# mousecpn/Boosting-R-CNN

Hardware: AMD Instinct MI355X
Metric: images/sec (1333x800) Boosting R-CNN R50-PAFPN inference (higher is better)
Workload: dtype f32; 1 GPU; boosting_rcnn_r50_pafpn_1x_utdac.py inference (model(return_loss=False, rescale=True): device pass + result copy + bbox2result), batch 8 x 3x800x1344 per GPU, f32 MFMA conv stack, 1000 pre-NMS / 256 proposals per image, seeded synthetic weights; global_batch=8, parallelism=dp1

## Files before the change

boosting-r-cnn_amd/csrc/conv_common.h:

```cpp
#pragma once
#include "common.h"

namespace brcnn_conv {

typedef float f32x16 __attribute__((ext_vector_type(16)));
typedef float f32x4 __attribute__((ext_vector_type(4)));
typedef unsigned int u32x4 __attribute__((ext_vector_type(4)));

constexpr int OOB = 0x7fffffff;

constexpr int BK = 32, LDS_STRIDE = 36;

struct ConvParams {
    const float* x;
    const float* w;
    const float* scale;
    const float* shift;
    const float* residual;
    float* y;
    int batch, Cin, Cout, KH, KW, stride, pad;
    int M, K;
    int relu;
    int tiles_m, tiles_n;
    int pitch;
// ... 78 lines not shown
    return r;
}
template <int ET> __device__ __forceinline__ unsigned brcnn_pk2(brcnn_f32x2 v) { return ET ? brcnn_pk2h(v.x, v.y) : brcnn_pk2b(v.x, v.y); }
__device__ __forceinline__ unsigned brcnn_relu_pk(unsigned w, unsigned floor2) {
    const brcnn_i16x2 a = __builtin_bit_cast(brcnn_i16x2, w), f = __builtin_bit_cast(brcnn_i16x2, floor2);
    return __builtin_bit_cast(unsigned, __builtin_elementwise_max(a, f));
}

int conv1x1_stream_try(ConvParams& p, hipStream_t s, int f16);
int dispatch_conv_bf16(ConvParams& p, hipStream_t s);
int dispatch_conv_pp_bf16(ConvParams& p, hipStream_t s);
int dispatch_conv_pp128_bf16(ConvParams& p, hipStream_t s);
int sk_plan_pp(ConvParams& p, int slots, int bm, int bn, hipStream_t s);
int sk_plan_pp_f32(ConvParams& p, int slots, int bm, int bn, hipStream_t s);
int sk_plan_f32_tile(ConvParams& p, int per_cu, int cus, hipStream_t s);
float* conv_ws_wgrad_slabs(hipStream_t s);
float* wgrad_defer_slabs(hipStream_t s, size_t bytes, int* err);
void wgrad_defer_push(hipStream_t s, float* slab, float* dw, int tiles, int tiles_k, int slices, int group, int Cout, int K,
                      int kind);
unsigned* conv_ws_wgrad_counters(hipStream_t s);
int wgrad_pp_bf16_try(const void* x, const void* dy, void* dw, int batch, int num_segments, const int* heights_host,
                      const int* widths_host, int cin, int cout, int kh, int kw, int stride, int pad, hipStream_t stream,
                      int f16);
int dispatch_conv_pp_f32(ConvParams& p, hipStream_t s);

}
```

boosting-r-cnn_amd/csrc/conv_igemm_bf16.hip:

```cpp
#include <algorithm>
#include <mutex>
#include <vector>
#include "conv_common.h"
#include "policy.h"

namespace {
using namespace brcnn_conv;

typedef __bf16 bf16x8 __attribute__((ext_vector_type(8)));
typedef _Float16 f16x8 __attribute__((ext_vector_type(8)));
typedef __attribute__((address_space(3))) void* lds_ptr_t;
constexpr int BKE = 64;

__device__ __forceinline__ unsigned short f2bf(float v) { return brcnn_f2b(v); }
__device__ __forceinline__ float bf2f(unsigned short h) { return __uint_as_float(((unsigned)h) << 16); }
template <int ET> __device__ __forceinline__ float e2f(unsigned short h) { return ET ? brcnn_h2f(h) : bf2f(h); }
template <int ET> __device__ __forceinline__ unsigned short f2e(float v) { return ET ? brcnn_f2h(v) : f2bf(v); }
template <int ET> __device__ __forceinline__ unsigned pk2e(float lo, float hi) { return ET ? brcnn_pk2h(lo, hi) : brcnn_pk2b(lo, hi); }

template <int MT, int NT, bool RES, bool OUTF32, int WM, int WNW = 2, int ST = 2, int ET = 0, int MODE = 0, bool SK = false>
__global__ __launch_bounds__(64 * WM * WNW, (ST == 2 && MT * NT <= 4 && (WM * WNW == 4 || MT == 1)) ? 2 : 1) void conv_igemm_bf16_dma_kernel(ConvParams p) {
    constexpr int NW = WNW * WM;
    constexpr int BM = 32 * MT * WM, BN = 32 * NT * WNW;
    constexpr int AG = BM / 8 / NW;
// ... 1118 lines not shown
    const long long tiles = (long long)p.tiles_m * p.tiles_n;
    const int nk = p.K / 32;
    if (nk < 2 || (p.K % 32) || tiles < slots || tiles * nk >= 0x7fffffffLL) return 0;
    if ((size_t)slots * 64 * 64 * sizeof(float) > SK_WS_BYTES) return 0;
    std::lock_guard<std::mutex> lock(g_sk_mutex);
    SkStream* st = nullptr;
    int rc = sk_stream_state(s, &st);
    if (rc) return rc;
    const SkTable* tab = nullptr;
    rc = sk_table_ranges(tiles, nk, slots, &tab);
    if (rc) return rc == BRCNN_EINVAL ? 0 : rc;
    sk_fill(p, *st, *tab);
    return 0;
}

static int dispatch_conv_f16(ConvParams& p, hipStream_t s) {
    p.il = 0;
    if (brcnn::g_policy.bf16_tile == 0) {
        if (const int rc = conv1x1_stream_try(p, s, 1)) return rc < 0 ? rc : 0;
    }
    if (p.gstep) return launch2<1, 1, 4, 2, 2, 1>(p, s);
    if (brcnn::g_policy.bf16_tile == 8842 && pp128_ok(p)) return dispatch_conv_pp128_bf16(p, s);
    if (brcnn::g_policy.bf16_tile == 8844 && pp_ok(p)) return dispatch_conv_pp_bf16(p, s);
    if (pp128_wins(p)) return dispatch_conv_pp128_bf16(p, s);
    if (pp_wins(p)) return dispatch_conv_pp_bf16(p, s);
    const long long t22 = (long long)((p.M + 127) / 128) * ((p.Cout + 127) / 128);
    const long long t44 = (long long)((p.M + 255) / 256) * ((p.Cout + 255) / 256);
    const bool fill44 = p.Cout >= 256 && p.K >= 1024 && !p.residual && !p.out_f32 && !p.z_out && !p.tail_z && t44 >= 512 &&
                        (double)t44 / (double)(((t44 + 255) / 256) * 256) >= 0.85;
    if (fill44 && p.Cout > 128) return launch2<2, 2, 4, 4, 2, 1>(p, s);
// ... 62 lines not shown
```

boosting-r-cnn_amd/csrc/conv_winograd_f32.hip:

```cpp
#include "conv_common.h"
#include "policy.h"

namespace {
using namespace brcnn_conv;

typedef __attribute__((address_space(3))) void* lds_ptr_t;

struct WinoSegs {
    int nseg, batch;
    int H[BRCNN_MAX_LEVELS], W[BRCNN_MAX_LEVELS], TH[BRCNN_MAX_LEVELS], TW[BRCNN_MAX_LEVELS];
    int t0[BRCNN_MAX_LEVELS + 1];
    int r0[BRCNN_MAX_LEVELS + 1];
};

struct WinoTile { int seg, n, h, w; };
__device__ __forceinline__ WinoTile wino_tile(const WinoSegs& sg, int t) {
    int s = 0;
#pragma unroll
    for (int i = 1; i < BRCNN_MAX_LEVELS; i++)
        if (i < sg.nseg && t >= sg.t0[i]) s = i;
    const int l = t - sg.t0[s];
    const int per = sg.TH[s] * sg.TW[s];
    const int n = l / per, rem = l - n * per;
    const int th = rem / sg.TW[s];
// ... 90 lines not shown
#pragma unroll
        for (int b = 0; b < 4; b++)
            *reinterpret_cast<float4*>(vs + (size_t)(a * 4 + b) * xi_stride) = make_float4(d[a][b][0], d[a][b][1], d[a][b][2], d[a][b][3]);
}

struct WinoGemmParams {
    const float* v;
    const float* u;
    const float* scale;
    const float* shift;
    float* y;
    unsigned v_bytes, u_bytes;
    int tile0, nt, Cin, Cout, relu;
    int tiles_m, tiles_n;
    WinoSegs sg;
};

constexpr int WBM_MAX = 64;

__device__ __forceinline__ constexpr int wino_at(int a, int i) { return a == 0 ? (i < 3 ? 1 : 0) : (i == 0 ? 0 : (i == 1 ? 1 : -1)); }

template <int WBM, int WBN, int WNW>
__global__ __launch_bounds__(256, 2) void wino_gemm_kernel(WinoGemmParams p) {
#if defined(__HIP_DEVICE_COMPILE__)
    constexpr int NB = WBN / (32 * WNW);
    static_assert(WBM % 32 == 0 && (WBM / 32) * WNW == 4 && NB * 32 * WNW == WBN && (NB == 1 || NB == 2), "four waves of 32 x 32 NB");
    static_assert(2 * WBM * 32 + 2 * WBN * 32 >= 4 * 1024, "the read-out slabs live in the staging buffers");
    __shared__ __attribute__((aligned(16))) float smem[2 * WBM * 32 + 2 * WBN * 32];
    float* As = smem;
    float* Bs = smem + 2 * WBM * 32;
    const int tid = threadIdx.x;
    const int lane = tid & 63;
    const int wave = __builtin_amdgcn_readfirstlane(tid >> 6);
    const int wm = wave / WNW, wn = wave % WNW;
    const int li = lane & 31, lh = lane >> 5;

    const int tile = xcd_remap(blockIdx.x, p.tiles_m * p.tiles_n);
    const int tile_m = tile / p.tiles_n, tile_n = tile - tile_m * p.tiles_n;
    const int m0 = tile_m * WBM, n0 = tile_n * WBN;

    const __amdgpu_buffer_rsrc_t rsrc_v = __builtin_amdgcn_make_buffer_rsrc((void*)p.v, 0, (int)p.v_bytes, 0x00020000);
    const __amdgpu_buffer_rsrc_t rsrc_u = __builtin_amdgcn_make_buffer_rsrc((void*)p.u, 0, (int)p.u_bytes, 0x00020000);

    constexpr int AG = WBM / 8 / 4, BG = WBN / 8 / 4;
    const int rg = lane >> 3, pc = lane & 7;
    int a_off[AG], b_off[BG];
#pragma unroll
    for (int j = 0; j < AG; j++) {
        const int r = (wave * AG + j) * 8 + rg;
        const int t = m0 + r;
        a_off[j] = t < p.nt ? (t * p.Cin + (pc ^ ((r >> 1) & 7)) * 4) * 4 : -1;
    }
#pragma unroll
    for (int j = 0; j < BG; j++) {
        const int r = (wave * BG + j) * 8 + rg;
        const int co = n0 + r;
        b_off[j] = co < p.Cout ? (co * p.Cin + (pc ^ ((r >> 1) & 7)) * 4) * 4 : -1;
    }
    const int nk = p.Cin / 32;
    const int a_xi = p.nt * p.Cin * 4, b_xi = p.Cout * p.Cin * 4;
    int s_xi = 0, s_kc = 0;
    auto dma_step = [&](int buf) {
        const int ao = s_xi * a_xi + s_kc * 128, bo = s_xi * b_xi + s_kc * 128;
        if (++s_kc == nk) { s_kc = 0; s_xi++; }
#pragma unroll
        for (int j = 0; j < AG; j++) {
            float* dst = As + buf * WBM * 32 + (wave * AG + j) * 8 * 32;
            __builtin_amdgcn_raw_ptr_buffer_load_lds(rsrc_v, (lds_ptr_t)dst, 16, a_off[j] >= 0 ? a_off[j] + ao : OOB, 0, 0, 0);
        }
#pragma unroll
        for (int j = 0; j < BG; j++) {
            float* dst = Bs + buf * WBN * 32 + (wave * BG + j) * 8 * 32;
            __builtin_amdgcn_raw_ptr_buffer_load_lds(rsrc_u, (lds_ptr_t)dst, 16, b_off[j] >= 0 ? b_off[j] + bo : OOB, 0, 0, 0);
        }
    };

// ... 13 lines not shown
        if constexpr (NB == 2)
            asm volatile("s_waitcnt lgkmcnt(0)" : "+v"(av[slot]), "+v"(bv[slot][0]), "+v"(bv[slot][NB - 1]) :: "memory");
        else
            asm volatile("s_waitcnt lgkmcnt(0)" : "+v"(av[slot]), "+v"(bv[slot][0]) :: "memory");
    };

    f32x16 yacc[4][NB], tmp[NB];
#pragma unroll
    for (int q = 0; q < 4; q++)
#pragma unroll
        for (int b = 0; b < NB; b++)
#pragma unroll
            for (int r = 0; r < 16; r++) yacc[q][b][r] = 0.f;

    dma_step(0);
    asm volatile("s_waitcnt vmcnt(0)" ::: "memory");
    __syncthreads();
    int cur = 0;
    for (int xi = 0; xi < 16; xi++) {
#pragma unroll
        for (int b = 0; b < NB; b++)
#pragma unroll
            for (int r = 0; r < 16; r++) tmp[b][r] = 0.f;
        for (int kc = 0; kc < nk; kc++) {
            const unsigned a_cur = a_lane + cur * (WBM * 32 * 4);
            const unsigned b_cur = b_lane + cur * (WBN * 32 * 4);
            frag_read(0, a_cur + chb[0], b_cur + chb[0]);
            if (xi < 15 || kc + 1 < nk) dma_step(cur ^ 1);
            frag_wait(0);
#pragma unroll
            for (int kk = 0; kk < 4; kk++) {
                const int sl = kk & 1;
                if (kk + 1 < 4) frag_read(sl ^ 1, a_cur + chb[kk + 1], b_cur + chb[kk + 1]);
#pragma unroll
                for (int e = 0; e < 4; e++)
#pragma unroll
                    for (int b = 0; b < NB; b++)
                        tmp[b] = __builtin_amdgcn_mfma_f32_32x32x2f32(av[sl][e], bv[sl][b][e], tmp[b], 0, 0, 0);
                if (kk + 1 < 4) frag_wait(sl ^ 1);
            }
            asm volatile("s_waitcnt vmcnt(0)" ::: "memory");
            __syncthreads();
            cur ^= 1;
        }
        const int i = xi >> 2, j = xi & 3;
#pragma unroll
        for (int a = 0; a < 2; a++)
#pragma unroll
            for (int bq = 0; bq < 2; bq++) {
                const float c = (float)(wino_at(a, i) * wino_at(bq, j));
#pragma unroll
                for (int b = 0; b < NB; b++)
#pragma unroll
                    for (int r = 0; r < 16; r++) yacc[a * 2 + bq][b][r] = __builtin_fmaf(c, tmp[b][r], yacc[a * 2 + bq][b][r]);
            }
    }

    float* slab = smem + wave * 1024;
    const int vrow = lane >> 3, vcol = (lane & 7) * 4;
    long long prow[4];
    int pw[4], pflag[4];
#pragma unroll
    for (int it = 0; it < 4; it++) {
        const int tl = m0 + wm * 32 + it * 8 + vrow;
        prow[it] = -1; pw[it] = 0; pflag[it] = 0;
        if (tl < p.nt) {
            const WinoTile t = wino_tile(p.sg, p.tile0 + tl);
            const int H = p.sg.H[t.seg], W = p.sg.W[t.seg];
            prow[it] = ((long long)p.sg.r0[t.seg] + ((long long)t.n * H + t.h) * W + t.w) * p.Cout;
            pw[it] = W;
// ... 17 lines not shown
                slab[((r & 3) + 8 * (r >> 2) + 4 * lh) * 32 + li] = o + sh;
            }
            __builtin_amdgcn_s_waitcnt(0xc07f);
            __builtin_amdgcn_wave_barrier();
#pragma unroll
            for (int it = 0; it < 4; it++) {
                float4 o = *reinterpret_cast<const float4*>(slab + (it * 8 + vrow) * 32 + vcol);
                if (p.relu) { o.x = fmaxf(o.x, 0.f); o.y = fmaxf(o.y, 0.f); o.z = fmaxf(o.z, 0.f); o.w = fmaxf(o.w, 0.f); }
                const bool in_map = ((q & 1) == 0 || (pflag[it] & 1)) && ((q & 2) == 0 || (pflag[it] & 2));
                if (prow[it] >= 0 && in_map && cv < p.Cout)
                    *reinterpret_cast<float4*>(yout + prow[it] + (long long)((q >> 1) * pw[it] + (q & 1)) * p.Cout + cv) = o;
            }
            __builtin_amdgcn_s_waitcnt(0xc07f);
            __builtin_amdgcn_wave_barrier();
        }
    }
#endif
}

int wino_segs(WinoSegs& sg, int batch, int num_segments, const int* heights_host, const int* widths_host) {
    if (batch <= 0 || num_segments <= 0 || num_segments > BRCNN_MAX_LEVELS || !heights_host || !widths_host) return BRCNN_EINVAL;
    sg = {};
    sg.nseg = num_segments;
    sg.batch = batch;
    long long tiles = 0, rows = 0;
    for (int s = 0; s < num_segments; s++) {
        const int H = heights_host[s], W = widths_host[s];
        if (H <= 0 || W <= 0 || H >= 4096 || W >= 4096) return BRCNN_EINVAL;
        sg.H[s] = H; sg.W[s] = W; sg.TH[s] = (H + 1) / 2; sg.TW[s] = (W + 1) / 2;
        sg.t0[s] = (int)tiles; sg.r0[s] = (int)rows;
// ... 13 lines not shown
    if (cin <= 0 || wino_segs(sg, batch, num_segments, heights_host, widths_host)) return 0;
    return (size_t)16 * (size_t)sg.t0[num_segments] * (size_t)cin * sizeof(float);
}

BRCNN_API int brcnn_winograd_filter_f32(const void* w, void* u, int cout, int cin, int kh, int kw, int dtype, void* stream) {
    if (!w || !u || dtype != BRCNN_DT_F32 || kh != 3 || kw != 3 || cin <= 0 || cout <= 0 || (cin % 32) || (cout % 64) ||
        (long long)cout * cin * 64 >= 0x7fffffffLL)
        return BRCNN_EINVAL;
    hipLaunchKernelGGL(wino_filter_kernel, dim3((cout * cin + 255) / 256), dim3(256), 0, (hipStream_t)stream, (const float*)w,
                       (float*)u, cout, cin);
    BRCNN_LAUNCH_CHECK();
    return 0;
}

namespace {

int wino_run(const void* x, const void* u, const void* gn_stats, const float* gamma, const float* beta, int groups, int relu_in,
             const float* scale, const float* shift, int relu, void* y, void* workspace, size_t workspace_bytes, WinoGemmParams& p,
             int num_segments, int cin, int cout, int variant, void* stream) {
    const int tiles = p.sg.t0[num_segments];
    if ((long long)p.sg.r0[num_segments] * (cin > cout ? cin : cout) * 4 >= 0x7fffffffLL) return BRCNN_EINVAL;
    if (workspace_bytes < (size_t)16 * tiles * cin * sizeof(float)) return BRCNN_EINVAL;
    const int wbm = variant == 2 ? 32 : 64, wbn = variant == 3 ? 64 : 128;
    int chunks = brcnn::g_policy.f32_winograd_chunks;
    while ((long long)16 * ((tiles + chunks - 1) / chunks + WBM_MAX) * cin * 4 >= 0x7fffffffLL) chunks *= 2;
    const int per = ((tiles + chunks - 1) / chunks + WBM_MAX - 1) / WBM_MAX * WBM_MAX;
    hipStream_t s = (hipStream_t)stream;
    p.v = (const float*)workspace; p.u = (const float*)u; p.scale = scale; p.shift = shift; p.y = (float*)y;
    p.u_bytes = (unsigned)((long long)cout * cin * 64);
    p.Cin = cin; p.Cout = cout; p.relu = relu;
    p.tiles_n = (cout + wbn - 1) / wbn;
    for (int t0 = 0; t0 < tiles; t0 += per) {
        const int nt = tiles - t0 < per ? tiles - t0 : per;
        const long long th = (long long)nt * (cin >> 2);
        hipLaunchKernelGGL(wino_input_kernel, dim3((unsigned)((th + 255) / 256)), dim3(256), 0, s, (const float*)x, (float*)workspace,
                           p.sg, t0, nt, cin, (const double*)gn_stats, gamma, beta, groups, relu_in);
        BRCNN_LAUNCH_CHECK();
        p.tile0 = t0; p.nt = nt;
        p.v_bytes = (unsigned)((long long)16 * nt * cin * 4);
        p.tiles_m = (nt + wbm - 1) / wbm;
        const dim3 grid(p.tiles_m * p.tiles_n);
        if (variant == 2) hipLaunchKernelGGL((wino_gemm_kernel<32, 128, 4>), grid, dim3(256), 0, s, p);
        else if (variant == 3) hipLaunchKernelGGL((wino_gemm_kernel<64, 64, 2>), grid, dim3(256), 0, s, p);
        else hipLaunchKernelGGL((wino_gemm_kernel<64, 128, 2>), grid, dim3(256), 0, s, p);
        BRCNN_LAUNCH_CHECK();
    }
    return 0;
}

}

BRCNN_API int brcnn_conv3x3_winograd_f32_multi(const void* x, const void* u, const void* gn_stats, const float* gamma,
                                               const float* beta, int groups, int relu_in, const float* scale,
                                               const float* shift, int relu, void* y, void* workspace, size_t workspace_bytes,
                                               int batch, int num_segments, const int* heights_host, const int* widths_host,
                                               int cin, int cout, int kh, int kw, int stride, int pad, int dtype, void* stream) {
    if (!x || !u || !y || !workspace || dtype != BRCNN_DT_F32 || kh != 3 || kw != 3 || stride != 1 || pad != 1 || cin <= 0 ||
        cout <= 0 || (cin % 32) || (cout % 64) || (long long)cout * cin * 64 >= 0x7fffffffLL)
        return BRCNN_EINVAL;
    if (gn_stats && (!gamma || !beta || groups <= 0 || cin % groups)) return BRCNN_EINVAL;
    WinoGemmParams p = {};
    if (wino_segs(p.sg, batch, num_segments, heights_host, widths_host)) return BRCNN_EINVAL;
    const int st = wino_run(x, u, gn_stats, gamma, beta, groups, relu_in, scale, shift, relu, y, workspace, workspace_bytes, p,
                            num_segments, cin, cout, 1, stream);
    if (st) return st;
    brcnn::count(brcnn::g_counters.f32_winograd_launches);
    brcnn::g_counters.f32_winograd_tiles = p.sg.t0[num_segments];
    return 0;
}

BRCNN_API int brcnn_conv3x3_winograd_f32_layer(const void* x, const void* u, const float* scale, const float* shift, int relu,
                                               void* y, void* workspace, size_t workspace_bytes, int batch, int height, int width,
                                               int cin, int cout, int kh, int kw, int stride, int pad, int dtype, void* stream) {
    if (!x || !u || !y || !workspace || dtype != BRCNN_DT_F32 || kh != 3 || kw != 3 || stride != 1 || pad != 1 || cin <= 0 ||
        cout <= 0 || (cin % 32) || (cout % 64) || (long long)cout * cin * 64 >= 0x7fffffffLL)
        return BRCNN_EINVAL;
    WinoGemmParams p = {};
    if (wino_segs(p.sg, batch, 1, &height, &width)) return BRCNN_EINVAL;
    const int variant = brcnn::wino_gemm_variant(p.sg.t0[1], cout);
    const int st = wino_run(x, u, nullptr, nullptr, nullptr, 0, 0, scale, shift, relu, y, workspace, workspace_bytes, p, 1, cin,
                            cout, variant, stream);
    if (st) return st;
// ... 5 lines not shown
```

boosting-r-cnn_amd/csrc/policy.h:

```cpp
#pragma once

namespace brcnn {

struct Policy {
    int use_dma = 1;
    int force_wm = 0, force_nt = 0;
    int no_fast = 0;
    int pp_f32_n128 = 1;
    int pp_f32_mode = 1;
    int f32_tile_sk = 1;
    int f32_tile_sk_per_cu = 0;
    int f32_winograd = 1;
    int f32_winograd_chunks = 1;
    int f32_winograd_layer = 1;
    int f32_winograd_gemm = 0;

    int dcn_fused = 1;

    int bf16_tile = 0;
    int bf16_il = 0;
    int sk_mode = 1;
    int sk_par = 0;
    int pp_mode = 1;
    int pp128_mode = 1;
    int pp128_min_k = 4096;
    int pp128_max_t88 = 128;
    int sk_spin_limit = 1 << 24;
    int sk_drop_publish = 0;
    int stream_mode = 1;

// ... 28 lines not shown
    int stream1x1_launches = 0;
    int sk_chain_fills = 0;
    int sk_par_fills = 0;
    int sk_last_wgs = 0;
    int bf16_tile_launches = 0;
    int bf16_tile_rows = 0;
    int bf16_tile_cols = 0;
    int bf16_tile_waves = 0;
    int bf16_tile_stages = 0;
    int wgrad_bf16_tile_launches = 0;
    int wgrad_bf16_last_tile = 0;
    int f32_winograd_launches = 0;
    int f32_winograd_tiles = 0;
    int f32_winograd_layer_launches = 0;
    int f32_winograd_layer_variant = 0;
    int dcn_fused_launches = 0;
    int dcn_im2col_launches = 0;
    int roi_ordered_launches = 0;
    int roi_prepared_launches = 0;
    int roi_gather_chunked = 0;
    int roi_gather_last_ch = 0;
};
extern Counters g_counters;
inline void count(int& c) { c = (c + 1) & 0x7fffffff; }

int wino_layer_rule(int tiles, int cin, int cout);
int wino_gemm_rule(int tiles, int cout);
int wino_gemm_variant(int tiles, int cout);

}
```

boosting-r-cnn_amd/csrc/policy.hip:

```cpp
#include "common.h"
#include "policy.h"

__attribute__((require_constant_initialization)) brcnn::Policy brcnn::g_policy;
__attribute__((require_constant_initialization)) brcnn::Counters brcnn::g_counters;
using brcnn::g_counters, brcnn::g_policy;

BRCNN_API int brcnn_conv_set_tile(int wm, int nt) {
    if (wm == -1) { g_policy.use_dma = nt; return 0; }
    if (wm == -3) { if (nt < 0 || nt > 2) return BRCNN_EINVAL; g_policy.pp_f32_n128 = nt; return 0; }
    if (wm == -4) { if (nt != 0 && nt != 1) return BRCNN_EINVAL; g_policy.no_fast = nt; return 0; }
    if (wm == -5) { if (nt < 0 || nt > 2) return BRCNN_EINVAL; g_policy.f32_tile_sk = nt; return 0; }
    if (wm == -7) { if (nt < 0 || nt > 8) return BRCNN_EINVAL; g_policy.f32_tile_sk_per_cu = nt; return 0; }
    if (wm == -6) return nt == 0 ? g_counters.f32_tile_sk_launches : nt == 1 ? g_counters.f32_tile_sk_wgs : BRCNN_EINVAL;
    if (wm == -9) {
        int* const c[] = {&g_counters.pp_f32_launches, &g_counters.pp_f32_rows, &g_counters.pp_f32_cols, &g_counters.pp_bf16_launches,
                          &g_counters.pp128_bf16_launches, &g_counters.stream1x1_launches, &g_counters.sk_chain_fills,
                          &g_counters.sk_par_fills, &g_counters.sk_last_wgs, &g_counters.bf16_tile_launches, &g_counters.bf16_tile_rows,
                          &g_counters.bf16_tile_cols, &g_counters.bf16_tile_waves, &g_counters.bf16_tile_stages,
                          &g_counters.wgrad_bf16_tile_launches, &g_counters.wgrad_bf16_last_tile};
        const int count = (int)(sizeof(c) / sizeof(c[0]));
        if (nt < -1 || nt >= count) return BRCNN_EINVAL;
        if (nt == -1) {
            for (int* q : c) *q = 0;
            g_counters.f32_winograd_launches = g_counters.f32_winograd_tiles = 0;
            g_counters.dcn_fused_launches = g_counters.dcn_im2col_launches = 0;
            g_counters.f32_winograd_layer_launches = g_counters.f32_winograd_layer_variant = 0;
            return 0;
        }
        const int n = *c[nt];
        *c[nt] = 0;
        return n;
    }
    if (wm == -11) {
        if (nt == 0 || nt == 1) { g_policy.f32_winograd = nt; return 0; }
        if (nt == 2) return g_policy.f32_winograd;
        if (nt >= 11 && nt <= 18) { g_policy.f32_winograd_chunks = nt - 10; return 0; }
        return BRCNN_EINVAL;
    }
    if (wm == -12) {
        if (nt != 0 && nt != 1) return BRCNN_EINVAL;
        int& c = nt == 0 ? g_counters.f32_winograd_launches : g_counters.f32_winograd_tiles;
// ... 9 lines not shown
        const int n = c;
        c = 0;
        return n;
    }
    if (wm == -14) {
        if (nt >= 0 && nt <= 2) { g_policy.f32_winograd_layer = nt; return 0; }
        if (nt == 3) return g_policy.f32_winograd_layer;
        if (nt >= 20 && nt <= 23) { g_policy.f32_winograd_gemm = nt - 20; return 0; }
        if (nt == 24) return g_policy.f32_winograd_gemm;
        if (nt != 10 && nt != 11) return BRCNN_EINVAL;
        int& c = nt == 10 ? g_counters.f32_winograd_layer_launches : g_counters.f32_winograd_layer_variant;
        const int n = c;
        c = 0;
        return n;
    }
    if (wm == -2) { if (nt != 0 && nt != 1 && nt != 2 && nt != 128 && nt != 256) return BRCNN_EINVAL; g_policy.pp_f32_mode = nt; return 0; }
    if ((wm != 0 && wm != 1 && wm != 2 && wm != 4) || nt < 0 || nt > 2) return BRCNN_EINVAL;
    g_policy.force_wm = wm;
    g_policy.force_nt = nt;
    return 0;
}

int brcnn::wino_gemm_rule(int tiles, int cout) {
    (void)tiles; (void)cout;
    return 3;
}

int brcnn::wino_layer_rule(int tiles, int cin, int cout) {
    if (cin != cout) return 0;
    if (cin == 256) return tiles >= 5250;
    if (cin == 512) return tiles >= 444;
    return 0;
}

int brcnn::wino_gemm_variant(int tiles, int cout) {
    return g_policy.f32_winograd_gemm ? g_policy.f32_winograd_gemm : wino_gemm_rule(tiles, cout);
}

BRCNN_API int brcnn_winograd_layer_route(int tiles, int cin, int cout, int kh, int kw, int stride, int pad, int dilation,
                                         int groups, int dtype) {
    if (tiles <= 0 || cin <= 0 || cout <= 0 || kh != 3 || kw != 3 || stride != 1 || pad != 1 || dilation != 1 || groups != 1 ||
        (cin % 32) || (cout % 64) || dtype != BRCNN_DT_F32 || (long long)cout * cin * 64 >= 0x7fffffffLL)
        return 0;
    if (!g_policy.f32_winograd || !g_policy.f32_winograd_layer) return 0;
    if (g_policy.f32_winograd_layer == 2) return 1;
    return brcnn::wino_layer_rule(tiles, cin, cout);
}

BRCNN_API int brcnn_winograd_layer_gemm_variant(int tiles, int cout) { return brcnn::wino_gemm_variant(tiles, cout); }

BRCNN_API int brcnn_conv_set_tile_bf16(int mtnt) {
// ... 97 lines not shown
```

boosting-r-cnn_amd/lib.py:

```python
import ctypes
import os

_HERE = os.path.dirname(os.path.abspath(__file__))
LIB_PATH = os.environ.get('BRCNN_LIB_PATH') or os.path.join(_HERE, 'lib', 'libbrcnn_hip.so')
_lib = None

c_int, c_i64, c_f32, c_f64, c_ptr, c_size = (ctypes.c_int, ctypes.c_int64, ctypes.c_float,
                                             ctypes.c_double, ctypes.c_void_p, ctypes.c_size_t)

SIGNATURES = {
    'brcnn_version': (c_int, []),
    'brcnn_device_count': (c_int, []),
    'brcnn_roi_align_forward': (c_int, [c_ptr] * 5 + [c_int] * 7 + [c_f32] + [c_int] * 4 + [c_ptr]),
    'brcnn_roi_align_backward': (c_int, [c_ptr] * 3 + [c_int] * 7 + [c_f32] + [c_int] * 3 + [c_ptr]),
    'brcnn_roi_extract_forward': (c_int, [c_ptr] * 4 + [c_int] + [c_ptr] * 3 + [c_int] * 6 +
                                  [c_f32, c_int, c_ptr]),
    'brcnn_roi_extract_forward_ordered': (c_int, [c_ptr] * 4 + [c_int] + [c_ptr] * 3 + [c_int] * 6 +
                                          [c_f32, c_int, c_ptr, c_ptr]),
    'brcnn_roi_extract_prep_workspace_bytes': (c_size, [c_int]),
    'brcnn_roi_extract_order_min_rois': (c_int, []),
    'brcnn_roi_extract_forward_prepared': (c_int, [c_ptr] * 4 + [c_int] + [c_ptr] * 3 + [c_int] * 6 +
                                           [c_f32, c_int, c_ptr, c_ptr, c_size, c_ptr]),
    'brcnn_get_tuning': (c_int, [c_ptr]),
    'brcnn_set_tuning': (c_int, [c_ptr]),
# ... 16 lines not shown
    'brcnn_conv2d_nhwc': (c_int, [c_ptr] * 6 + [c_int] * 11 + [c_ptr]),
    'brcnn_conv_set_tile': (c_int, [c_int, c_int]),
    'brcnn_clock_probe': (c_int, [c_ptr, c_i64, c_ptr]),
    'brcnn_nms_prepare': (c_int, [c_ptr] * 9 + [c_int, c_int, c_ptr]),
    'brcnn_nms_collect': (c_int, [c_ptr] * 7 + [c_int, c_int, c_int, c_ptr]),
    'brcnn_conv2d_nhwc_scatter2': (c_int, [c_ptr] * 3 + [c_int] * 14 + [c_ptr]),
    'brcnn_conv2d_nhwc_multi': (c_int, [c_ptr] * 6 + [c_int, c_int, c_ptr, c_ptr] + [c_int] * 8 +
                                [c_ptr]),
    'brcnn_winograd_filter_f32': (c_int, [c_ptr, c_ptr] + [c_int] * 5 + [c_ptr]),
    'brcnn_conv3x3_winograd_f32_multi_workspace_bytes': (c_size, [c_int, c_int, c_ptr, c_ptr, c_int]),
    'brcnn_conv3x3_winograd_f32_multi': (c_int, [c_ptr] * 5 + [c_int, c_int, c_ptr, c_ptr, c_int, c_ptr, c_ptr, c_size,
                                                 c_int, c_int, c_ptr, c_ptr] + [c_int] * 7 + [c_ptr]),
    'brcnn_conv3x3_winograd_f32_layer': (c_int, [c_ptr] * 4 + [c_int, c_ptr, c_ptr, c_size] + [c_int] * 10 + [c_ptr]),
    'brcnn_winograd_layer_route': (c_int, [c_int] * 10),
    'brcnn_winograd_layer_gemm_variant': (c_int, [c_int, c_int]),
    'brcnn_groupnorm_nhwc_multi_stats': (c_int, [c_ptr, c_ptr, c_int, c_int, c_ptr, c_int, c_int, c_f32, c_int, c_ptr]),
    'brcnn_conv2d_dgrad_nhwc_multi': (c_int, [c_ptr] * 3 + [c_int, c_int] + [c_ptr] * 4 + [c_int] * 7 +
                                      [c_ptr]),
    'brcnn_conv2d_wgrad_nhwc_multi': (c_int, [c_ptr] * 3 + [c_int, c_int] + [c_ptr] * 2 + [c_int] * 7 +
                                      [c_ptr]),
    'brcnn_wgrad_defer_begin': (c_int, [c_ptr, c_ptr, c_size, c_int]),
    'brcnn_wgrad_defer_flush': (c_int, [c_ptr]),
    'brcnn_wgrad_defer_pending': (c_int, [c_ptr]),
    'brcnn_wgrad_defer_stats': (c_int, [c_ptr, c_ptr, c_ptr]),
    'brcnn_stem_workspace_bytes': (c_size, [c_int, c_int, c_int]),
    'brcnn_stem7x7s2_nchw': (c_int, [c_ptr] * 6 + [c_int] * 6 + [c_ptr]),
    'brcnn_stem7x7s2_pool_nchw': (c_int, [c_ptr] * 5 + [c_int] * 5 + [c_ptr]),
    'brcnn_bottleneck_tail_f32': (c_int, [c_ptr] * 9 + [c_int] * 3 + [c_ptr]),
    'brcnn_bottleneck_tail_16': (c_int, [c_ptr] * 9 + [c_int] * 4 + [c_ptr]),
    'brcnn_conv_set_tile_bf16': (c_int, [c_int]),
# ... 202 lines not shown
```

include/brcnn_hip.h:

```cpp
#ifndef BRCNN_HIP_H
#define BRCNN_HIP_H

#include <stddef.h>
#include <stdint.h>

#ifdef __cplusplus
extern "C" {
#endif

#define BRCNN_LAYOUT_NCHW 0
#define BRCNN_LAYOUT_NHWC 1

#define BRCNN_DT_F32 0
#define BRCNN_DT_BF16 1
#define BRCNN_DT_BF16_OUT_F32 2
#define BRCNN_DT_F16 3
#define BRCNN_DT_F16_OUT_F32 4

#define BRCNN_MAX_LEVELS 8
#define BRCNN_MAX_IMAGES 64

int brcnn_version(void);

int brcnn_clock_probe(int64_t *out2, int64_t wall_ticks_100mhz, void *stream);
// ... 141 lines not shown
int brcnn_winograd_filter_f32(const void *w, void *u, int cout, int cin, int kh, int kw, int dtype, void *stream);
size_t brcnn_conv3x3_winograd_f32_multi_workspace_bytes(int batch, int num_segments, const int *heights_host,
                                                        const int *widths_host, int cin);
int brcnn_conv3x3_winograd_f32_multi(const void *x, const void *u, const void *gn_stats, const float *gamma,
                                     const float *beta, int groups, int relu_in, const float *scale,
                                     const float *shift, int relu, void *y, void *workspace, size_t workspace_bytes,
                                     int batch, int num_segments, const int *heights_host, const int *widths_host,
                                     int cin, int cout, int kh, int kw, int stride, int pad, int dtype, void *stream);

int brcnn_conv3x3_winograd_f32_layer(const void *x, const void *u, const float *scale, const float *shift, int relu,
                                     void *y, void *workspace, size_t workspace_bytes, int batch, int height, int width,
                                     int cin, int cout, int kh, int kw, int stride, int pad, int dtype, void *stream);
int brcnn_winograd_layer_route(int tiles, int cin, int cout, int kh, int kw, int stride, int pad, int dilation,
                               int groups, int dtype);
int brcnn_winograd_layer_gemm_variant(int tiles, int cout);

int brcnn_conv2d_nhwc_grouped(const void *x, const void *w_tiles, const float *scale,
                              const float *shift, const void *residual, void *y, int batch,
                              int height, int width, int cin, int cout, int kh, int kw, int stride,
                              int pad, int window, int relu, int dtype, void *stream);
int brcnn_conv2d_dgrad_nhwc_grouped(const void *dy, const void *w_t_tiles, void *dx, int batch,
                                    int in_height, int in_width, int out_height, int out_width, int cin,
                                    int cout, int kh, int kw, int stride, int pad, int window, int dtype,
                                    void *stream);
int brcnn_conv2d_wgrad_nhwc_grouped(const void *x, const void *dy, void *dw_tiles, int batch, int height,
                                    int width, int cin, int cout, int kh, int kw, int stride, int pad,
                                    int window, int dtype, void *stream);

int brcnn_conv2d_dgrad_nhwc_multi(const void *dy, const void *w_t, void *dx, int batch,
                                  int num_segments, const int *in_heights_host,
// ... 321 lines not shown
```

Measured before the change: 394.3 images/sec.

## Add stream-K persistent scheduling and optional three-stage ring to Winograd f32 GEMM

```diff
diff --git a/boosting-r-cnn_amd/csrc/conv_common.h b/boosting-r-cnn_amd/csrc/conv_common.h
--- a/boosting-r-cnn_amd/csrc/conv_common.h
+++ b/boosting-r-cnn_amd/csrc/conv_common.h
@@ -116,6 +116,8 @@
 int sk_plan_pp(ConvParams& p, int slots, int bm, int bn, hipStream_t s);
 int sk_plan_pp_f32(ConvParams& p, int slots, int bm, int bn, hipStream_t s);
 int sk_plan_f32_tile(ConvParams& p, int per_cu, int cus, hipStream_t s);
+struct SkRangePlan { int wgs; const int4* items; float* ws; unsigned* flags; unsigned epoch; unsigned* err; int spin_limit; };
+int sk_plan_ranges(SkRangePlan& k, long long tiles, int nk, int slots, size_t slot_bytes, hipStream_t s);
 float* conv_ws_wgrad_slabs(hipStream_t s);
 float* wgrad_defer_slabs(hipStream_t s, size_t bytes, int* err);
 void wgrad_defer_push(hipStream_t s, float* slab, float* dw, int tiles, int tiles_k, int slices, int group, int Cout, int K,
diff --git a/boosting-r-cnn_amd/csrc/conv_igemm_bf16.hip b/boosting-r-cnn_amd/csrc/conv_igemm_bf16.hip
--- a/boosting-r-cnn_amd/csrc/conv_igemm_bf16.hip
+++ b/boosting-r-cnn_amd/csrc/conv_igemm_bf16.hip
@@ -1156,6 +1156,27 @@
     return 0;
 }
 
+int sk_plan_ranges(SkRangePlan& k, long long tiles, int nk, int slots, size_t slot_bytes, hipStream_t s) {
+    k = {};
+    if (int e = sk_take_error()) return e;
+    if (brcnn::g_policy.sk_mode == 0 || slots <= 0 || slots > SK_MAX_SLOTS) return 0;
+    if (sk_capturing(s)) return 0;
+    if (nk < 2 || tiles < slots || tiles * nk >= 0x7fffffffLL) return 0;
+    if ((size_t)slots * slot_bytes > SK_WS_BYTES) return 0;
+    std::lock_guard<std::mutex> lock(g_sk_mutex);
+    SkStream* st = nullptr;
+    int rc = sk_stream_state(s, &st);
+    if (rc) return rc;
+    const SkTable* tab = nullptr;
+    rc = sk_table_ranges(tiles, nk, slots, &tab);
+    if (rc) return rc == BRCNN_EINVAL ? 0 : rc;
+    ConvParams p = {};
+    sk_fill(p, *st, *tab);
+    k.wgs = p.sk_wgs; k.items = p.sk_items; k.ws = p.sk_ws; k.flags = p.sk_flags; k.epoch = p.sk_epoch; k.err = p.sk_err;
+    k.spin_limit = p.sk_spin_limit;
+    return 0;
+}
+
 static int dispatch_conv_f16(ConvParams& p, hipStream_t s) {
     p.il = 0;
     if (brcnn::g_policy.bf16_tile == 0) {
diff --git a/boosting-r-cnn_amd/csrc/conv_winograd_f32.hip b/boosting-r-cnn_amd/csrc/conv_winograd_f32.hip
--- a/boosting-r-cnn_amd/csrc/conv_winograd_f32.hip
+++ b/boosting-r-cnn_amd/csrc/conv_winograd_f32.hip
@@ -128,28 +128,32 @@
     int tile0, nt, Cin, Cout, relu;
     int tiles_m, tiles_n;
     WinoSegs sg;
+    const int4* sk_items;
+    float* sk_ws;
+    unsigned* sk_flags;
+    unsigned sk_epoch;
+    unsigned* sk_err;
+    int sk_spin_limit;
 };
 
 constexpr int WBM_MAX = 64;
 
 __device__ __forceinline__ constexpr int wino_at(int a, int i) { return a == 0 ? (i < 3 ? 1 : 0) : (i == 0 ? 0 : (i == 1 ? 1 : -1)); }
 
-template <int WBM, int WBN, int WNW>
-__global__ __launch_bounds__(256, 2) void wino_gemm_kernel(WinoGemmParams p) {
+template <int WBM, int WBN, int WNW, bool PERS, int RING>
+__device__ __forceinline__ void wino_gemm_item(const WinoGemmParams& p, float* smem, const int tile, const int xb_, const int xe_,
+                                               const int slot) {
 #if defined(__HIP_DEVICE_COMPILE__)
     constexpr int NB = WBN / (32 * WNW);
-    static_assert(WBM % 32 == 0 && (WBM / 32) * WNW == 4 && NB * 32 * WNW == WBN && (NB == 1 || NB == 2), "four waves of 32 x 32 NB");
-    static_assert(2 * WBM * 32 + 2 * WBN * 32 >= 4 * 1024, "the read-out slabs live in the staging buffers");
-    __shared__ __attribute__((aligned(16))) float smem[2 * WBM * 32 + 2 * WBN * 32];
+    const int xb = PERS ? xb_ : 0, xe = PERS ? xe_ : 16;
     float* As = smem;
-    float* Bs = smem + 2 * WBM * 32;
+    float* Bs = smem + RING * WBM * 32;
     const int tid = threadIdx.x;
     const int lane = tid & 63;
     const int wave = __builtin_amdgcn_readfirstlane(tid >> 6);
     const int wm = wave / WNW, wn = wave % WNW;
     const int li = lane & 31, lh = lane >> 5;
 
-    const int tile = xcd_remap(blockIdx.x, p.tiles_m * p.tiles_n);
     const int tile_m = tile / p.tiles_n, tile_n = tile - tile_m * p.tiles_n;
     const int m0 = tile_m * WBM, n0 = tile_n * WBN;
 
@@ -173,7 +177,7 @@
     }
     const int nk = p.Cin / 32;
     const int a_xi = p.nt * p.Cin * 4, b_xi = p.Cout * p.Cin * 4;
-    int s_xi = 0, s_kc = 0;
+    int s_xi = xb, s_kc = 0;
     auto dma_step = [&](int buf) {
         const int ao = s_xi * a_xi + s_kc * 128, bo = s_xi * b_xi + s_kc * 128;
         if (++s_kc == nk) { s_kc = 0; s_xi++; }
@@ -217,19 +221,76 @@
             for (int r = 0; r < 16; r++) yacc[q][b][r] = 0.f;
 
     dma_step(0);
+    if constexpr (RING == 3) {
+        if ((xe - xb) * nk > 1) dma_step(1);
+    }
+    if constexpr (PERS) {
+        if (xb > 0) {
+            if (tid == 0) {
+                int spins = 0;
+                while (__hip_atomic_load(p.sk_flags + slot, __ATOMIC_RELAXED, __HIP_MEMORY_SCOPE_AGENT) != p.sk_epoch &&
+                       ++spins < p.sk_spin_limit)
+                    __builtin_amdgcn_s_sleep(4);
+                if (spins >= p.sk_spin_limit)
+                    __hip_atomic_store(p.sk_err, p.sk_epoch | 0x80000000u, __ATOMIC_RELAXED, __HIP_MEMORY_SCOPE_SYSTEM);
+                __builtin_amdgcn_fence(__ATOMIC_ACQUIRE, "agent");
+            }
+            __syncthreads();
+            const f32x4* src = reinterpret_cast<const f32x4*>(p.sk_ws) + (size_t)slot * (WBM * WBN) + wave * 64 + lane;
+#pragma unroll
+            for (int q = 0; q < 4; q++)
+#pragma unroll
+                for (int b = 0; b < NB; b++)
+#pragma unroll
+                    for (int g = 0; g < 4; g++) {
+                        const f32x4 v = src[((q * NB + b) * 4 + g) * 256];
+                        yacc[q][b][4 * g + 0] = v.x; yacc[q][b][4 * g + 1] = v.y;
+                        yacc[q][b][4 * g + 2] = v.z; yacc[q][b][4 * g + 3] = v.w;
+                    }
+#pragma unroll
+            for (int q = 0; q < 4; q++)
+#pragma unroll
+                for (int b = 0; b < NB; b++) asm volatile("" : "+v"(yacc[q][b]));
+        }
+    }
     asm volatile("s_waitcnt vmcnt(0)" ::: "memory");
     __syncthreads();
     int cur = 0;
-    for (int xi = 0; xi < 16; xi++) {
+    [[maybe_unused]] int left = (xe - xb) * nk;
+    for (int xi = xb; xi < xe; xi++) {
 #pragma unroll
         for (int b = 0; b < NB; b++)
 #pragma unroll
             for (int r = 0; r < 16; r++) tmp[b][r] = 0.f;
+        if constexpr (RING == 3) {
+            for (int kc = 0; kc < nk; kc++, left--) {
+                if (left > 1) asm volatile("s_waitcnt vmcnt(%0)" ::"n"(AG + BG) : "memory");
+                else asm volatile("s_waitcnt vmcnt(0)" ::: "memory");
+                __syncthreads();
+                const unsigned a_cur = a_lane + cur * (WBM * 32 * 4);
+                const unsigned b_cur = b_lane + cur * (WBN * 32 * 4);
+                frag_read(0, a_cur + chb[0], b_cur + chb[0]);
+                if (left > 2) dma_step(cur == 0 ? 2 : cur - 1);
+                frag_wait(0);
+#pragma unroll
+                for (int kk = 0; kk < 4; kk++) {
+                    const int sl = kk & 1;
+                    if (kk + 1 < 4) frag_read(sl ^ 1, a_cur + chb[kk + 1], b_cur + chb[kk + 1]);
+#pragma unroll
+                    for (int e = 0; e < 4; e++)
+#pragma unroll
+                        for (int b = 0; b < NB; b++)
+                            tmp[b] = __builtin_amdgcn_mfma_f32_32x32x2f32(av[sl][e], bv[sl][b][e], tmp[b], 0, 0, 0);
+                    if (kk + 1 < 4) frag_wait(sl ^ 1);
+                }
+                cur = cur == 2 ? 0 : cur + 1;
+            }
+        } else
         for (int kc = 0; kc < nk; kc++) {
             const unsigned a_cur = a_lane + cur * (WBM * 32 * 4);
             const unsigned b_cur = b_lane + cur * (WBN * 32 * 4);
             frag_read(0, a_cur + chb[0], b_cur + chb[0]);
-            if (xi < 15 || kc + 1 < nk) dma_step(cur ^ 1);
+            if (xi < xe - 1 || kc + 1 < nk) dma_step(cur ^ 1);
             frag_wait(0);
 #pragma unroll
             for (int kk = 0; kk < 4; kk++) {
@@ -257,6 +318,32 @@
 #pragma unroll
                     for (int r = 0; r < 16; r++) yacc[a * 2 + bq][b][r] = __builtin_fmaf(c, tmp[b][r], yacc[a * 2 + bq][b][r]);
             }
+    }
+
+    if constexpr (RING == 3) __syncthreads();
+    if constexpr (PERS) {
+        if (xe < 16) {
+            f32x4* dst = reinterpret_cast<f32x4*>(p.sk_ws) + (size_t)slot * (WBM * WBN) + wave * 64 + lane;
+#pragma unroll
+            for (int q = 0; q < 4; q++)
+#pragma unroll
+                for (int b = 0; b < NB; b++)
+#pragma unroll
+                    for (int g = 0; g < 4; g++) {
+                        f32x4 v;
+                        v.x = yacc[q][b][4 * g + 0]; v.y = yacc[q][b][4 * g + 1];
+                        v.z = yacc[q][b][4 * g + 2]; v.w = yacc[q][b][4 * g + 3];
+                        dst[((q * NB + b) * 4 + g) * 256] = v;
+                    }
+            asm volatile("s_waitcnt vmcnt(0)" ::: "memory");
+            __syncthreads();
+            if (tid == 0) {
+                __builtin_amdgcn_fence(__ATOMIC_RELEASE, "agent");
+                asm volatile("s_waitcnt vmcnt(0)" ::: "memory");
+                __hip_atomic_store(p.sk_flags + slot, p.sk_epoch, __ATOMIC_RELAXED, __HIP_MEMORY_SCOPE_AGENT);
+            }
+            return;
+        }
     }
 
     float* slab = smem + wave * 1024;
@@ -304,6 +391,29 @@
             __builtin_amdgcn_s_waitcnt(0xc07f);
             __builtin_amdgcn_wave_barrier();
         }
+    }
+#endif
+}
+
+template <int WBM, int WBN, int WNW, bool PERS = false, int RING = 2>
+__global__ __launch_bounds__(256, 2) void wino_gemm_kernel(WinoGemmParams p) {
+#if defined(__HIP_DEVICE_COMPILE__)
+    static_assert(WBM % 32 == 0 && (WBM / 32) * WNW == 4 && (WBN == 32 * WNW || WBN == 64 * WNW), "four waves of 32 x 32 NB");
+    static_assert(RING == 2 || RING == 3, "two or three LDS stages");
+    static_assert(RING * (WBM * 32 + WBN * 32) >= 4 * 1024, "the read-out slabs live in the staging buffers");
+    __shared__ __attribute__((aligned(16))) float smem[RING * (WBM * 32 + WBN * 32)];
+    if constexpr (PERS) {
+        const int4 range = p.sk_items[blockIdx.x];
+        const int first = __builtin_amdgcn_readfirstlane(range.x), count = __builtin_amdgcn_readfirstlane(range.y);
+        for (int i = 0; i < count; i++) {
+            if (i > 0) __syncthreads();
+            const int4 item = p.sk_items[first + i];
+            wino_gemm_item<WBM, WBN, WNW, true, RING>(p, smem, __builtin_amdgcn_readfirstlane(item.x),
+                                                __builtin_amdgcn_readfirstlane(item.y), __builtin_amdgcn_readfirstlane(item.z),
+                                                __builtin_amdgcn_readfirstlane(item.w));
+        }
+    } else {
+        wino_gemm_item<WBM, WBN, WNW, false, RING>(p, smem, xcd_remap(blockIdx.x, p.tiles_m * p.tiles_n), 0, 16, 0);
     }
 #endif
 }
@@ -347,6 +457,64 @@
 }
 
 namespace {
+
+int g_wino_cus = 0;
+template <int WBM, int WBN, int WNW, int RING>
+int wino_occupancy(int& occ) {
+    static int cached = -1;
+    if (cached < 0) {
+        int n = 0;
+        BRCNN_HIP_CHECK(hipOccupancyMaxActiveBlocksPerMultiprocessor(&n, (const void*)wino_gemm_kernel<WBM, WBN, WNW, true, RING>, 256, 0));
+        if (g_wino_cus == 0) {
+            int dev = 0;
+            hipDeviceProp_t prop;
+            BRCNN_HIP_CHECK(hipGetDevice(&dev));
+            BRCNN_HIP_CHECK(hipGetDeviceProperties(&prop, dev));
+            g_wino_cus = prop.multiProcessorCount;
+        }
+        cached = n;
+    }
+    occ = cached;
+    return 0;
+}
+
+template <int RING>
+int wino_occupancy_of(int variant, int& occ) {
+    return variant == 2 ? wino_occupancy<32, 128, 4, RING>(occ) : variant == 3 ? wino_occupancy<64, 64, 2, RING>(occ)
+                                                                               : wino_occupancy<64, 128, 2, RING>(occ);
+}
+
+int wino_plan(WinoGemmParams& p, int variant, int ring, hipStream_t s, int& wgs) {
+    wgs = 0;
+    const int mode = brcnn::g_policy.f32_winograd_sk;
+    if (mode == 0) return 0;
+    int occ = 0;
+    if (const int rc = ring == 3 ? wino_occupancy_of<3>(variant, occ) : wino_occupancy_of<2>(variant, occ)) return rc;
+    const int cus = g_wino_cus;
+    const long long tiles = (long long)p.tiles_m * p.tiles_n;
+    int per_cu = occ;
+    if (brcnn::g_policy.f32_winograd_sk_per_cu > 0 && brcnn::g_policy.f32_winograd_sk_per_cu < per_cu) per_cu = brcnn::g_policy.f32_winograd_sk_per_cu;
+    if (per_cu <= 0 || cus <= 0) return 0;
+    if (tiles < (long long)per_cu * cus) per_cu = tiles / cus > 1 ? (int)(tiles / cus) : 1;
+    if (mode == 1 && !brcnn::wino_persistent_rule(tiles > 0x7fffffffLL ? 0x7fffffff : (int)tiles, 16, cus, per_cu)) return 0;
+    long long slots = (long long)per_cu * cus;
+    if (brcnn::g_policy.f32_winograd_sk_wgs > 0 && brcnn::g_policy.f32_winograd_sk_wgs < slots) slots = brcnn::g_policy.f32_winograd_sk_wgs;
+    const int wbm = variant == 2 ? 32 : 64, wbn = variant == 3 ? 64 : 128;
+    SkRangePlan k;
+    if (const int rc = sk_plan_ranges(k, tiles, 16, (int)slots, (size_t)4 * wbm * wbn * sizeof(float), s)) return rc;
+    if (k.wgs <= 0) return 0;
+    p.sk_items = k.items; p.sk_ws = k.ws; p.sk_flags = k.flags; p.sk_epoch = k.epoch; p.sk_err = k.err;
+    p.sk_spin_limit = k.spin_limit;
+    wgs = k.wgs;
+    return 0;
+}
+
+template <bool PERS, int RING>
+void wino_launch(int variant, const dim3& grid, hipStream_t s, const WinoGemmParams& p) {
+    if (variant == 2) hipLaunchKernelGGL((wino_gemm_kernel<32, 128, 4, PERS, RING>), grid, dim3(256), 0, s, p);
+    else if (variant == 3) hipLaunchKernelGGL((wino_gemm_kernel<64, 64, 2, PERS, RING>), grid, dim3(256), 0, s, p);
+    else hipLaunchKernelGGL((wino_gemm_kernel<64, 128, 2, PERS, RING>), grid, dim3(256), 0, s, p);
+}
 
 int wino_run(const void* x, const void* u, const void* gn_stats, const float* gamma, const float* beta, int groups, int relu_in,
              const float* scale, const float* shift, int relu, void* y, void* workspace, size_t workspace_bytes, WinoGemmParams& p,
@@ -372,10 +540,22 @@
         p.tile0 = t0; p.nt = nt;
         p.v_bytes = (unsigned)((long long)16 * nt * cin * 4);
         p.tiles_m = (nt + wbm - 1) / wbm;
+        const int ring = brcnn::g_policy.f32_winograd_ring ? brcnn::g_policy.f32_winograd_ring
+                                                           : brcnn::wino_ring_rule(p.tiles_m * p.tiles_n, cin);
+        brcnn::g_counters.f32_winograd_last_ring = ring;
+        int wgs = 0;
+        if (const int rc = wino_plan(p, variant, ring, s, wgs)) return rc;
+        if (wgs > 0) {
+            if (ring == 3) wino_launch<true, 3>(variant, dim3(wgs), s, p);
+            else wino_launch<true, 2>(variant, dim3(wgs), s, p);
+            BRCNN_LAUNCH_CHECK();
+            brcnn::count(brcnn::g_counters.f32_winograd_sk_launches);
+            brcnn::g_counters.f32_winograd_sk_last_wgs = wgs;
+            continue;
+        }
         const dim3 grid(p.tiles_m * p.tiles_n);
-        if (variant == 2) hipLaunchKernelGGL((wino_gemm_kernel<32, 128, 4>), grid, dim3(256), 0, s, p);
-        else if (variant == 3) hipLaunchKernelGGL((wino_gemm_kernel<64, 64, 2>), grid, dim3(256), 0, s, p);
-        else hipLaunchKernelGGL((wino_gemm_kernel<64, 128, 2>), grid, dim3(256), 0, s, p);
+        if (ring == 3) wino_launch<false, 3>(variant, grid, s, p);
+        else wino_launch<false, 2>(variant, grid, s, p);
         BRCNN_LAUNCH_CHECK();
     }
     return 0;
@@ -394,11 +574,14 @@
     if (gn_stats && (!gamma || !beta || groups <= 0 || cin % groups)) return BRCNN_EINVAL;
     WinoGemmParams p = {};
     if (wino_segs(p.sg, batch, num_segments, heights_host, widths_host)) return BRCNN_EINVAL;
+    const int variant = brcnn::g_policy.f32_winograd_tower_gemm ? brcnn::g_policy.f32_winograd_tower_gemm
+                                                                : brcnn::wino_tower_gemm_rule(p.sg.t0[num_segments], cout);
     const int st = wino_run(x, u, gn_stats, gamma, beta, groups, relu_in, scale, shift, relu, y, workspace, workspace_bytes, p,
-                            num_segments, cin, cout, 1, stream);
+                            num_segments, cin, cout, variant, stream);
     if (st) return st;
     brcnn::count(brcnn::g_counters.f32_winograd_launches);
     brcnn::g_counters.f32_winograd_tiles = p.sg.t0[num_segments];
+    brcnn::g_counters.f32_winograd_tower_variant = variant;
     return 0;
 }
 
diff --git a/boosting-r-cnn_amd/csrc/policy.h b/boosting-r-cnn_amd/csrc/policy.h
--- a/boosting-r-cnn_amd/csrc/policy.h
+++ b/boosting-r-cnn_amd/csrc/policy.h
@@ -14,6 +14,11 @@
     int f32_winograd_chunks = 1;
     int f32_winograd_layer = 1;
     int f32_winograd_gemm = 0;
+    int f32_winograd_sk = 1;
+    int f32_winograd_sk_per_cu = 0;
+    int f32_winograd_sk_wgs = 0;
+    int f32_winograd_ring = 0;
+    int f32_winograd_tower_gemm = 0;
 
     int dcn_fused = 1;
 
@@ -72,6 +77,10 @@
     int f32_winograd_tiles = 0;
     int f32_winograd_layer_launches = 0;
     int f32_winograd_layer_variant = 0;
+    int f32_winograd_sk_launches = 0;
+    int f32_winograd_sk_last_wgs = 0;
+    int f32_winograd_tower_variant = 0;
+    int f32_winograd_last_ring = 0;
     int dcn_fused_launches = 0;
     int dcn_im2col_launches = 0;
     int roi_ordered_launches = 0;
@@ -85,5 +94,8 @@
 int wino_layer_rule(int tiles, int cin, int cout);
 int wino_gemm_rule(int tiles, int cout);
 int wino_gemm_variant(int tiles, int cout);
+int wino_persistent_rule(int workgroup_tiles, int units, int cus, int per_cu);
+int wino_tower_gemm_rule(int tiles, int cout);
+int wino_ring_rule(int workgroup_tiles, int cin);
 
 }
diff --git a/boosting-r-cnn_amd/csrc/policy.hip b/boosting-r-cnn_amd/csrc/policy.hip
--- a/boosting-r-cnn_amd/csrc/policy.hip
+++ b/boosting-r-cnn_amd/csrc/policy.hip
@@ -25,6 +25,8 @@
             g_counters.f32_winograd_launches = g_counters.f32_winograd_tiles = 0;
             g_counters.dcn_fused_launches = g_counters.dcn_im2col_launches = 0;
             g_counters.f32_winograd_layer_launches = g_counters.f32_winograd_layer_variant = 0;
+            g_counters.f32_winograd_sk_launches = g_counters.f32_winograd_sk_last_wgs = g_counters.f32_winograd_tower_variant = 0;
+            g_counters.f32_winograd_last_ring = 0;
             return 0;
         }
         const int n = *c[nt];
@@ -64,6 +66,24 @@
         c = 0;
         return n;
     }
+    if (wm == -16) {
+        if (nt >= 0 && nt <= 2) { g_policy.f32_winograd_sk = nt; return 0; }
+        if (nt == 3) return g_policy.f32_winograd_sk;
+        if (nt == 20 || nt == 21 || nt == 23) { g_policy.f32_winograd_tower_gemm = nt - 20; return 0; }
+        if (nt == 24) return g_policy.f32_winograd_tower_gemm;
+        if (nt >= 30 && nt <= 38) { g_policy.f32_winograd_sk_per_cu = nt - 30; return 0; }
+        if (nt == 39) return g_policy.f32_winograd_sk_per_cu;
+        if (nt == 40 || nt == 42 || nt == 43) { g_policy.f32_winograd_ring = nt - 40; return 0; }
+        if (nt == 49) return g_policy.f32_winograd_ring;
+        if (nt >= 1000 && nt <= 1000 + 2048) { g_policy.f32_winograd_sk_wgs = nt - 1000; return 0; }
+        if (nt == 999) return g_policy.f32_winograd_sk_wgs;
+        if (nt < 10 || nt > 13) return BRCNN_EINVAL;
+        int& c = nt == 10 ? g_counters.f32_winograd_sk_launches : nt == 11 ? g_counters.f32_winograd_sk_last_wgs
+                 : nt == 12 ? g_counters.f32_winograd_tower_variant : g_counters.f32_winograd_last_ring;
+        const int n = c;
+        c = 0;
+        return n;
+    }
     if (wm == -2) { if (nt != 0 && nt != 1 && nt != 2 && nt != 128 && nt != 256) return BRCNN_EINVAL; g_policy.pp_f32_mode = nt; return 0; }
     if ((wm != 0 && wm != 1 && wm != 2 && wm != 4) || nt < 0 || nt > 2) return BRCNN_EINVAL;
     g_policy.force_wm = wm;
@@ -85,6 +105,28 @@
 
 int brcnn::wino_gemm_variant(int tiles, int cout) {
     return g_policy.f32_winograd_gemm ? g_policy.f32_winograd_gemm : wino_gemm_rule(tiles, cout);
+}
+
+int brcnn::wino_persistent_rule(int workgroup_tiles, int units, int cus, int per_cu) {
+    if (workgroup_tiles <= 0 || units < 16 || cus <= 0 || per_cu <= 0) return 0;
+    const long long t256 = (long long)workgroup_tiles * 256;
+    if (per_cu == 1) return workgroup_tiles >= cus && t256 < 358LL * cus;
+    if (per_cu == 2) return t256 >= 520LL * cus && t256 < 584LL * cus;
+    return 0;
+}
+
+int brcnn::wino_ring_rule(int workgroup_tiles, int cin) {
+    (void)workgroup_tiles; (void)cin;
+    return 2;
+}
+
+int brcnn::wino_tower_gemm_rule(int tiles, int cout) {
+    (void)tiles; (void)cout;
+    return 1;
+}
+
+BRCNN_API int brcnn_winograd_persistent_rule(int workgroup_tiles, int units, int cus, int per_cu) {
+    return brcnn::wino_persistent_rule(workgroup_tiles, units, cus, per_cu);
 }
 
 BRCNN_API int brcnn_winograd_layer_route(int tiles, int cin, int cout, int kh, int kw, int stride, int pad, int dilation,
diff --git a/boosting-r-cnn_amd/lib.py b/boosting-r-cnn_amd/lib.py
--- a/boosting-r-cnn_amd/lib.py
+++ b/boosting-r-cnn_amd/lib.py
@@ -54,6 +54,7 @@
     'brcnn_conv3x3_winograd_f32_layer': (c_int, [c_ptr] * 4 + [c_int, c_ptr, c_ptr, c_size] + [c_int] * 10 + [c_ptr]),
     'brcnn_winograd_layer_route': (c_int, [c_int] * 10),
     'brcnn_winograd_layer_gemm_variant': (c_int, [c_int, c_int]),
+    'brcnn_winograd_persistent_rule': (c_int, [c_int] * 4),
     'brcnn_groupnorm_nhwc_multi_stats': (c_int, [c_ptr, c_ptr, c_int, c_int, c_ptr, c_int, c_int, c_f32, c_int, c_ptr]),
     'brcnn_conv2d_dgrad_nhwc_multi': (c_int, [c_ptr] * 3 + [c_int, c_int] + [c_ptr] * 4 + [c_int] * 7 +
                                       [c_ptr]),
diff --git a/include/brcnn_hip.h b/include/brcnn_hip.h
--- a/include/brcnn_hip.h
+++ b/include/brcnn_hip.h
@@ -179,6 +179,7 @@
 int brcnn_winograd_layer_route(int tiles, int cin, int cout, int kh, int kw, int stride, int pad, int dilation,
                                int groups, int dtype);
 int brcnn_winograd_layer_gemm_variant(int tiles, int cout);
+int brcnn_winograd_persistent_rule(int workgroup_tiles, int units, int cus, int per_cu);
 
 int brcnn_conv2d_nhwc_grouped(const void *x, const void *w_tiles, const float *scale,
                               const float *shift, const void *residual, void *y, int batch,
```

Measured after the change: 400.2 images/sec (median of 6 runs). 1.02x the previous value.
